# khuongnd6/ViT_torch

Hardware: AMD Instinct MI355X
Metric: images/sec fwd+bwd ViT-B/16 224^2 bs=256/GPU (higher is better)
Workload: dtype bf16; 1 GPU; dino_vitb16 224x224 fwd+CE+bwd+SGD(momentum) step, batch 256/GPU, 10 classes, random-init weights; global_batch=256, residual_stream=bf16, parallelism=dp1, hip_graph=True

## Files before the change

vit_torch_amd/csrc/common.h:

```cpp
#pragma once
#include <hip/hip_runtime.h>
#include <stdint.h>
#include <string>
#include "../../include/vitmi.h"

typedef __bf16 bf16;
typedef bf16 bf16x2 __attribute__((ext_vector_type(2)));
typedef bf16 bf16x4 __attribute__((ext_vector_type(4)));
typedef bf16 bf16x8 __attribute__((ext_vector_type(8)));
typedef float f32x2 __attribute__((ext_vector_type(2)));
typedef float f32x4 __attribute__((ext_vector_type(4)));
typedef float f32x16 __attribute__((ext_vector_type(16)));

#define LDS_PTR(T, p) ((__attribute__((address_space(3))) T*)(p))

void vitmi_set_error(const std::string& s);
int vitmi_fail(int code, const char* fmt, ...);
int vitmi_check_launch(const char* what);
int vitmi_cu_count();
int vitmi_persist_on(int launch_flags);
int vitmi_raise_dynamic_lds(const void* kern, int bytes, const char* who);
int vitmi_reduce_rows(const float* part, int S, int64_t N, int64_t ld, float* out, hipStream_t stream);
int vitmi_reduce_rows_segs(const float* part, int S, int64_t ld, float* const out[4], const int width[4],
                           hipStream_t stream);
int vitmi_reduce_rows3(const float* part, int S, int64_t N, int64_t ld, float* out0, float* out1, float* out2,
                       hipStream_t stream);

#define VITMI_REQUIRE(cond, code, ...)                  \
  do {                                                  \
    if (!(cond)) return vitmi_fail((code), __VA_ARGS__); \
  } while (0)

static inline bool is_aligned(const void* p, size_t a) {
  return (reinterpret_cast<uintptr_t>(p) % a) == 0;
}
static inline size_t dtype_size(int dt) { return dt == VITMI_BF16 ? 2 : 4; }

__device__ __forceinline__ float to_f32(float v) { return v; }
__device__ __forceinline__ float to_f32(bf16 v) { return (float)v; }
template <typename T> __device__ __forceinline__ T from_f32(float v);
template <> __device__ __forceinline__ float from_f32<float>(float v) { return v; }
template <> __device__ __forceinline__ bf16 from_f32<bf16>(float v) { return (bf16)v; }

__device__ __forceinline__ float wave_sum(float v) {
#pragma unroll
  for (int o = 32; o > 0; o >>= 1) v += __shfl_xor(v, o);
  return v;
}
__device__ __forceinline__ float wave_max(float v) {
#pragma unroll
  for (int o = 32; o > 0; o >>= 1) v = fmaxf(v, __shfl_xor(v, o));
  return v;
}

template <int CTRL, int ROW_MASK>
__device__ __forceinline__ float dpp_take(float old, float v) {
  return __builtin_bit_cast(float, __builtin_amdgcn_update_dpp(__builtin_bit_cast(int, old), __builtin_bit_cast(int, v),
                                                               CTRL, ROW_MASK, 0xf, false));
}
__device__ __forceinline__ float wave_sum_dpp(float v) {
  v += dpp_take<0xB1, 0xf>(0.f, v);
  v += dpp_take<0x4E, 0xf>(0.f, v);
  v += dpp_take<0x141, 0xf>(0.f, v);
  v += dpp_take<0x140, 0xf>(0.f, v);
  v += dpp_take<0x142, 0xa>(0.f, v);
  v += dpp_take<0x143, 0xc>(0.f, v);
  return __builtin_bit_cast(float, __builtin_amdgcn_readlane(__builtin_bit_cast(int, v), 63));
}
__device__ __forceinline__ float wave_max_dpp(float v) {
  v = fmaxf(v, dpp_take<0xB1, 0xf>(-INFINITY, v));
  v = fmaxf(v, dpp_take<0x4E, 0xf>(-INFINITY, v));
  v = fmaxf(v, dpp_take<0x141, 0xf>(-INFINITY, v));
  v = fmaxf(v, dpp_take<0x140, 0xf>(-INFINITY, v));
  v = fmaxf(v, dpp_take<0x142, 0xa>(-INFINITY, v));
  v = fmaxf(v, dpp_take<0x143, 0xc>(-INFINITY, v));
  return __builtin_bit_cast(float, __builtin_amdgcn_readlane(__builtin_bit_cast(int, v), 63));
}

__device__ __forceinline__ float gelu_erf(float x) {
  return 0.5f * x * (1.0f + erff(x * 0.70710678118654752440f));
}
__device__ __forceinline__ float dgelu_erf(float x) {
  const float cdf = 0.5f * (1.0f + erff(x * 0.70710678118654752440f));
  const float pdf = 0.39894228040143267794f * __expf(-0.5f * x * x);
  return cdf + x * pdf;
}

template <typename T> __device__ __forceinline__ f32x4 load4(const T* p);
template <> __device__ __forceinline__ f32x4 load4<float>(const float* p) {
  return *reinterpret_cast<const f32x4*>(p);
}
template <> __device__ __forceinline__ f32x4 load4<bf16>(const bf16* p) {
  bf16x4 v = *reinterpret_cast<const bf16x4*>(p);
  f32x4 r = {(float)v[0], (float)v[1], (float)v[2], (float)v[3]};
  return r;
}
template <typename T> __device__ __forceinline__ void store4(T* p, f32x4 v);
template <> __device__ __forceinline__ void store4<float>(float* p, f32x4 v) {
  *reinterpret_cast<f32x4*>(p) = v;
}
template <> __device__ __forceinline__ void store4<bf16>(bf16* p, f32x4 v) {
  bf16x4 r = {(bf16)v[0], (bf16)v[1], (bf16)v[2], (bf16)v[3]};
  *reinterpret_cast<bf16x4*>(p) = r;
}

__device__ __forceinline__ int mfma32_row(int reg, int lane_hi) {
  return (reg & 3) + 8 * (reg >> 2) + 4 * lane_hi;
}
```

vit_torch_amd/csrc/elementwise.hip:

```cpp
#include "common.h"

namespace {

constexpr int EW_BLOCK = 256;
inline unsigned ew_grid(int64_t work_items) {
  int64_t b = (work_items + EW_BLOCK - 1) / EW_BLOCK;
  const int64_t cap = 256 * 8;
  if (b > cap) b = cap;
  if (b < 1) b = 1;
  return (unsigned)b;
}

template <typename TS, typename TD>
__global__ void cast_kernel(const TS* __restrict__ src, TD* __restrict__ dst, int64_t n) {
  const int64_t stride = (int64_t)gridDim.x * blockDim.x;
  const int64_t n4 = n / 4;
  for (int64_t i = (int64_t)blockIdx.x * blockDim.x + threadIdx.x; i < n4; i += stride)
    store4<TD>(dst + i * 4, load4<TS>(src + i * 4));
  for (int64_t i = n4 * 4 + (int64_t)blockIdx.x * blockDim.x + threadIdx.x; i < n; i += stride)
    dst[i] = from_f32<TD>(to_f32(src[i]));
}

__global__ void axpy_kernel(const float* __restrict__ x, float* __restrict__ y, float a, int64_t n) {
  const int64_t stride = (int64_t)gridDim.x * blockDim.x;
// ... 168 lines not shown
  int n;
};
__global__ __launch_bounds__(1024) void fold_many_kernel(FoldTable t) {
  __shared__ float red[FOLD_GROUPS][FOLD_COLS];
  const int b = blockIdx.x;
  int i = 0;
  while (i < t.n - 1 && b >= t.blk_end[i]) ++i;
  const int lb = b - (i ? t.blk_end[i - 1] : 0);
  const int N = t.N[i], cb = (N + FOLD_COLS - 1) / FOLD_COLS;
  const int seg = lb / cb;
  const int64_t c = (int64_t)(lb % cb) * FOLD_COLS + threadIdx.x % FOLD_COLS;
  const float tot = fold_rows(t.part[i], t.S[i], t.ld[i], (int64_t)seg * N + c, c < N, red);
  if (threadIdx.x < FOLD_COLS && c < N) t.out[i][seg][c] = tot;
}

inline int colsum_splits(int64_t M) {
  int64_t s = (M + 3) / 4;
  return (int)(s < 512 ? s : 512);
}

constexpr float XENT_LSE_SWITCH = 16.f;
__global__ __launch_bounds__(256) void xent_kernel(const float* __restrict__ logits,
                                                   const int64_t* __restrict__ labels,
                                                   float* __restrict__ loss_rows,
                                                   float* __restrict__ dlogits,
                                                   int32_t* __restrict__ correct_rows,
                                                   int64_t B, int K) {
  const int lane = threadIdx.x & 63, w = threadIdx.x >> 6;
  const int64_t b = (int64_t)blockIdx.x * 4 + w;
  if (b >= B) return;
  const float* lr = logits + b * K;
  float mx = -INFINITY;
  int amax = 0;
  for (int k = lane; k < K; k += 64) {
    const float v = lr[k];
    if (v > mx) { mx = v; amax = k; }
  }
#pragma unroll
  for (int o = 32; o > 0; o >>= 1) {
    const float om = __shfl_xor(mx, o);
    const int oa = __shfl_xor(amax, o);
    if (om > mx || (om == mx && oa < amax)) { mx = om; amax = oa; }
  }
  float se = 0.f;
  for (int k = lane; k < K; k += 64) se += __expf(lr[k] - mx);
  se = wave_sum(se);
  const float lg = __logf(se);
  const float lse = mx + lg;
  const bool rel = !(fabsf(lse) < XENT_LSE_SWITCH);
  const int64_t lab = labels[b];
  const float invB = 1.f / (float)B;
  if (dlogits) {
    for (int k = lane; k < K; k += 64) {
      const float p = rel ? __expf((lr[k] - mx) - lg) : __expf(lr[k] - lse);
      dlogits[b * K + k] = (p - (k == lab ? 1.f : 0.f)) * invB;
    }
  }
  if (lane == 0) {
    const bool ok = lab >= 0 && lab < (int64_t)K;
    const float xl = lr[ok ? lab : 0];
    loss_rows[b] = ok ? (rel ? lg - (xl - mx) : lse - xl) : __builtin_nanf("");
    correct_rows[b] = (ok && amax == (int)lab) ? 1 : 0;
  }
}

__global__ __launch_bounds__(256) void xent_reduce_kernel(const float* __restrict__ loss_rows,
                                                          const int32_t* __restrict__ correct_rows,
                                                          float* __restrict__ loss,
                                                          int32_t* __restrict__ correct, int64_t B) {
  __shared__ float sl[256];
  __shared__ int sc[256];
  float l = 0.f;
  int c = 0;
  for (int64_t i = threadIdx.x; i < B; i += 256) { l += loss_rows[i]; c += correct_rows[i]; }
  sl[threadIdx.x] = l; sc[threadIdx.x] = c;
  __syncthreads();
  for (int o = 128; o > 0; o >>= 1) {
    if ((int)threadIdx.x < o) { sl[threadIdx.x] += sl[threadIdx.x + o]; sc[threadIdx.x] += sc[threadIdx.x + o]; }
    __syncthreads();
  }
  if (threadIdx.x == 0) { loss[0] = sl[0] / (float)B; if (correct) correct[0] = sc[0]; }
}

__global__ void sgd_momentum_kernel(float* __restrict__ p, const float* __restrict__ g,
                                    float* __restrict__ buf, bf16* __restrict__ shadow, int64_t n,
                                    float lr, float momentum, float gscale) {
  const int64_t stride = (int64_t)gridDim.x * blockDim.x;
  const int64_t n4 = n / 4;
  for (int64_t i = (int64_t)blockIdx.x * blockDim.x + threadIdx.x; i < n4; i += stride) {
    const f32x4 gv = __builtin_nontemporal_load(reinterpret_cast<const f32x4*>(g + i * 4));
    f32x4 bv = __builtin_nontemporal_load(reinterpret_cast<const f32x4*>(buf + i * 4));
    f32x4 pv = __builtin_nontemporal_load(reinterpret_cast<const f32x4*>(p + i * 4));
#pragma unroll
    for (int e = 0; e < 4; ++e) {
      bv[e] = momentum * bv[e] + gscale * gv[e];
      pv[e] = pv[e] - lr * bv[e];
    }
    __builtin_nontemporal_store(bv, reinterpret_cast<f32x4*>(buf + i * 4));
    __builtin_nontemporal_store(pv, reinterpret_cast<f32x4*>(p + i * 4));
    if (shadow) store4<bf16>(shadow + i * 4, pv);
  }
  for (int64_t i = n4 * 4 + (int64_t)blockIdx.x * blockDim.x + threadIdx.x; i < n; i += stride) {
    const float b = momentum * buf[i] + gscale * g[i];
    buf[i] = b;
    const float pn = p[i] - lr * b;
    p[i] = pn;
    if (shadow) shadow[i] = (bf16)pn;
  }
}

__global__ void adam_tick_kernel(float* state) { state[0] += 1.f; }

__global__ void adam_kernel(float* __restrict__ p, const float* __restrict__ g, float* __restrict__ m,
                            float* __restrict__ v, bf16* __restrict__ shadow, const float* __restrict__ state,
                            int64_t n, float lr, float b1, float b2, float eps, float wd, int decoupled,
                            float gscale) {
  const double t = state[0];
  const double bc1 = 1.0 - pow((double)b1, t), bc2 = 1.0 - pow((double)b2, t);
  const float step = (float)((double)lr / bc1), bc2s = (float)sqrt(bc2);
  const float lrwd = decoupled ? (float)((double)lr * (double)wd) : 0.f;
  const int64_t stride = (int64_t)gridDim.x * blockDim.x;
  for (int64_t i = (int64_t)blockIdx.x * blockDim.x + threadIdx.x; i < n; i += stride) {
    float pi = p[i], gi = g[i] * gscale;
    if (!decoupled) gi = fmaf(wd, pi, gi);
    const float mi = b1 * m[i] + (1.f - b1) * gi;
    const float vi = b2 * v[i] + (1.f - b2) * gi * gi;
    m[i] = mi;
    v[i] = vi;
    pi -= fmaf(lrwd, pi, step * mi / (sqrtf(vi) / bc2s + eps));
    p[i] = pi;
    if (shadow) shadow[i] = (bf16)pi;
  }
}

}

int vitmi_reduce_rows3(const float* part, int S, int64_t N, int64_t ld, float* out0, float* out1, float* out2,
                       hipStream_t stream) {
  const unsigned segs = out2 ? 3 : 2;
  hipLaunchKernelGGL(reduce_rows3_kernel, dim3((unsigned)((N + FOLD_COLS - 1) / FOLD_COLS), segs), dim3(1024), 0, stream, part, S,
                     N, ld, out0, out1, out2);
  return vitmi_check_launch("reduce_rows3_kernel");
}

int vitmi_reduce_rows_segs(const float* part, int S, int64_t ld, float* const out[4], const int width[4],
                           hipStream_t stream) {
  RowSegs sg;
  int e = 0;
  for (int i = 0; i < 4; ++i) { sg.out[i] = out[i]; e += width[i]; sg.end[i] = e; }
  hipLaunchKernelGGL(reduce_rows_segs_kernel, dim3((unsigned)((e + FOLD_COLS - 1) / FOLD_COLS)), dim3(1024), 0, stream, part, S, ld, sg);
  return vitmi_check_launch("reduce_rows_segs_kernel");
}

extern "C" int vitmi_fold_many(const vitmi_fold_desc* descs, int n, void* stream_) {
  VITMI_REQUIRE(descs && n > 0, VITMI_E_BADARG, "fold_many: null descriptors or n <= 0");
  hipStream_t stream = reinterpret_cast<hipStream_t>(stream_);
  for (int i0 = 0; i0 < n; i0 += FOLD_MAX) {
    FoldTable t;
    t.n = n - i0 < FOLD_MAX ? n - i0 : FOLD_MAX;
    int blocks = 0;
    for (int i = 0; i < FOLD_MAX; ++i) {
      const vitmi_fold_desc& d = descs[i0 + (i < t.n ? i : 0)];
      if (i < t.n) {
        VITMI_REQUIRE(d.struct_size == (int64_t)sizeof(vitmi_fold_desc), VITMI_E_BADARG, "fold_many: descriptor size %lld, this library expects %zu", (long long)d.struct_size, sizeof(vitmi_fold_desc));
        VITMI_REQUIRE(d.part && d.S > 0 && d.nseg >= 1 && d.nseg <= 3 && d.N > 0 && d.N < (1ll << 30) && d.ld >= d.nseg * d.N && d.ld < (1ll << 31),
                      VITMI_E_SHAPE, "fold_many: descriptor %d: S %d, nseg %d, N %lld, ld %lld", i0 + i, d.S, d.nseg, (long long)d.N, (long long)d.ld);
        for (int k = 0; k < d.nseg; ++k) VITMI_REQUIRE(d.out[k], VITMI_E_BADARG, "fold_many: descriptor %d: null output %d", i0 + i, k);
        blocks += d.nseg * (int)((d.N + FOLD_COLS - 1) / FOLD_COLS);
      }
      t.part[i] = d.part; t.S[i] = d.S; t.N[i] = (int)d.N; t.ld[i] = (int)d.ld; t.blk_end[i] = blocks;
      for (int k = 0; k < 3; ++k) t.out[i][k] = d.out[k < d.nseg ? k : 0];
    }
// ... 58 lines not shown
  if (out_ld <= 0) out_ld = C * p * p;
  VITMI_REQUIRE(out_ld >= C * p * p && out_ld % 4 == 0, VITMI_E_BADARG, "patchify: out_ld must be >= C*p*p and a multiple of 4");
  VITMI_REQUIRE(is_aligned(out, 4 * dtype_size(out_dtype)), VITMI_E_ALIGN, "patchify: out alignment");
  hipStream_t stream = reinterpret_cast<hipStream_t>(stream_);
  const int64_t ntok = cls_rows + (H / p) * (W / p);
  const int64_t total = B * ntok * (out_ld / 4);
  const unsigned grid = ew_grid(total);
  if (out_dtype == VITMI_BF16)
    hipLaunchKernelGGL((patchify_kernel<bf16>), dim3(grid), dim3(EW_BLOCK), 0, stream, x, sb, sc, sh, sw, (bf16*)out, out_ld, B, (int)C, (int)H, (int)W, (int)p, cls_rows);
  else if (out_dtype == VITMI_F32)
    hipLaunchKernelGGL((patchify_kernel<float>), dim3(grid), dim3(EW_BLOCK), 0, stream, x, sb, sc, sh, sw, (float*)out, out_ld, B, (int)C, (int)H, (int)W, (int)p, cls_rows);
  else return vitmi_fail(VITMI_E_DTYPE, "patchify: bad out dtype");
  return vitmi_check_launch("patchify_kernel");
}

extern "C" size_t vitmi_colsum_workspace(int64_t M, int64_t N) {
  return (size_t)colsum_splits(M) * (size_t)N * sizeof(float);
}

extern "C" int vitmi_colsum(const void* x, int dtype, int64_t M, int64_t N, int64_t ld, float* out,
                            void* workspace, size_t workspace_bytes, void* stream_) {
  VITMI_REQUIRE(x && out && M > 0 && N > 0 && ld >= N, VITMI_E_BADARG, "colsum: bad argument");
  VITMI_REQUIRE(workspace && workspace_bytes >= vitmi_colsum_workspace(M, N), VITMI_E_WORKSPACE, "colsum: workspace too small");
  hipStream_t stream = reinterpret_cast<hipStream_t>(stream_);
  if (dtype == VITMI_F32 && M <= 2048) return vitmi_reduce_rows(reinterpret_cast<const float*>(x), (int)M, N, ld, out, stream);
  const int S = colsum_splits(M);
  float* part = reinterpret_cast<float*>(workspace);
  const bool vec = (N % 4 == 0) && (ld % 4 == 0) && is_aligned(x, 4 * dtype_size(dtype));
  if (vec && N <= 512 && (dtype == VITMI_BF16 || dtype == VITMI_F32)) {
    const int gpr = (int)(N / 4);
    if (dtype == VITMI_BF16) hipLaunchKernelGGL((colsum_partial_rows_kernel<bf16>), dim3((unsigned)S), dim3(256), 0, stream, (const bf16*)x, M, gpr, ld, part);
    else hipLaunchKernelGGL((colsum_partial_rows_kernel<float>), dim3((unsigned)S), dim3(256), 0, stream, (const float*)x, M, gpr, ld, part);
    int rc = vitmi_check_launch("colsum_partial_rows_kernel");
    if (rc) return rc;
    return vitmi_reduce_rows(part, S, N, N, out, stream);
  }
  const int cols_per_block = vec ? 256 : 64;
  dim3 grid((unsigned)((N + cols_per_block - 1) / cols_per_block), (unsigned)S);
  if (dtype == VITMI_BF16) {
    if (vec) hipLaunchKernelGGL((colsum_partial_kernel<bf16, 4>), grid, dim3(256), 0, stream, (const bf16*)x, M, N, ld, part);
    else hipLaunchKernelGGL((colsum_partial_kernel<bf16, 1>), grid, dim3(256), 0, stream, (const bf16*)x, M, N, ld, part);
  } else if (dtype == VITMI_F32) {
    if (vec) hipLaunchKernelGGL((colsum_partial_kernel<float, 4>), grid, dim3(256), 0, stream, (const float*)x, M, N, ld, part);
    else hipLaunchKernelGGL((colsum_partial_kernel<float, 1>), grid, dim3(256), 0, stream, (const float*)x, M, N, ld, part);
  } else return vitmi_fail(VITMI_E_DTYPE, "colsum: bad dtype");
  int rc = vitmi_check_launch("colsum_partial_kernel");
  if (rc) return rc;
  return vitmi_reduce_rows(part, S, N, N, out, stream);
}

extern "C" int vitmi_softmax_xent(const float* logits, const int64_t* labels, float* loss,
                                  float* dlogits, int32_t* correct, int64_t B, int64_t K,
                                  void* stream_) {
  VITMI_REQUIRE(logits && labels && loss && B > 0 && K > 0, VITMI_E_BADARG, "softmax_xent: bad argument");
  VITMI_REQUIRE(dlogits, VITMI_E_BADARG, "softmax_xent: dlogits buffer required (its tail is used as scratch)");
  VITMI_REQUIRE(correct, VITMI_E_BADARG, "softmax_xent: correct buffer required");
  hipStream_t stream = reinterpret_cast<hipStream_t>(stream_);
  hipLaunchKernelGGL(xent_kernel, dim3((unsigned)((B + 3) / 4)), dim3(256), 0, stream, logits, labels, loss + 1, dlogits, correct + 1, B, (int)K);
  int rc = vitmi_check_launch("xent_kernel");
  if (rc) return rc;
  hipLaunchKernelGGL(xent_reduce_kernel, dim3(1), dim3(256), 0, stream, loss + 1, correct + 1, loss, correct, B);
  return vitmi_check_launch("xent_reduce_kernel");
}

extern "C" int vitmi_adam(float* p, const float* g, float* m, float* v, void* shadow, float* state, int64_t n,
                          float lr, float beta1, float beta2, float eps, float weight_decay, int decoupled,
                          float grad_scale, void* stream_) {
  VITMI_REQUIRE(p && g && m && v && state && n > 0, VITMI_E_BADARG, "adam: bad argument");
  VITMI_REQUIRE(beta1 >= 0.f && beta1 < 1.f && beta2 >= 0.f && beta2 < 1.f && eps >= 0.f, VITMI_E_BADARG, "adam: bad hyper-parameter");
  hipStream_t stream = reinterpret_cast<hipStream_t>(stream_);
  hipLaunchKernelGGL(adam_tick_kernel, dim3(1), dim3(1), 0, stream, state);
  int rc = vitmi_check_launch("adam_tick_kernel");
  if (rc) return rc;
  hipLaunchKernelGGL(adam_kernel, dim3(ew_grid(n)), dim3(EW_BLOCK), 0, stream, p, g, m, v, (bf16*)shadow, state, n, lr,
                     beta1, beta2, eps, weight_decay, decoupled, grad_scale);
  return vitmi_check_launch("adam_kernel");
}

extern "C" int vitmi_sgd_momentum(float* p, const float* g, float* buf, void* shadow, int64_t n,
                                  float lr, float momentum, float grad_scale, void* stream_) {
  VITMI_REQUIRE(p && g && buf && n > 0, VITMI_E_BADARG, "sgd_momentum: bad argument");
  VITMI_REQUIRE(is_aligned(p, 16) && is_aligned(g, 16) && is_aligned(buf, 16) && (!shadow || is_aligned(shadow, 8)), VITMI_E_ALIGN, "sgd_momentum: buffers must be 16-B aligned");
  hipStream_t stream = reinterpret_cast<hipStream_t>(stream_);
  hipLaunchKernelGGL(sgd_momentum_kernel, dim3(ew_grid(n / 4 + 1)), dim3(EW_BLOCK), 0, stream, p, g, buf, (bf16*)shadow, n, lr, momentum, grad_scale);
  return vitmi_check_launch("sgd_momentum_kernel");
}
```

vit_torch_amd/csrc/layernorm.hip:

```cpp
#include <atomic>
#include <initializer_list>
#include "common.h"

namespace {

constexpr int LN_MAXV = 8;

template <int NV, typename TX, typename TY>
__global__ __launch_bounds__(256) void ln_fwd_kernel(const TX* __restrict__ x, int64_t xs,
                                                     const float* __restrict__ gamma,
                                                     const float* __restrict__ beta,
                                                     TY* __restrict__ y, int64_t ys,
                                                     float* __restrict__ mean_out,
                                                     float* __restrict__ rstd_out,
                                                     int64_t M, int D, float eps) {
  const int lane = threadIdx.x & 63, w = threadIdx.x >> 6;
  for (int64_t row = (int64_t)blockIdx.x * 4 + w; row < M; row += (int64_t)gridDim.x * 4) {
  const TX* xr = x + row * xs;
  f32x4 v[NV];
  float s = 0.f;
#pragma unroll
  for (int i = 0; i < NV; ++i) v[i] = load4<TX>(xr + min((i * 64 + lane) * 4, D - 4));
#pragma unroll
  for (int i = 0; i < NV; ++i) {
// ... 81 lines not shown
          dv[i][j] *= gam[i][j];
          s1 += dv[i][j];
          s2 += dv[i][j] * xh[i][j];
        }
      }
    }
    const float c1 = wave_sum(s1) * invD, c2 = wave_sum(s2) * invD;
    float rsc = 1.f;
    if (gb_rowscale) rsc = gb_rowscale[(uint32_t)row / (uint32_t)rpg];
    f32x4 gin[NV];
    if (g_in) {
#pragma unroll
      for (int i = 0; i < NV; ++i) gin[i] = load4<TG>(g_in + row * gstride + min((i * 64 + lane) * 4, D - 4));
    }
#pragma unroll
    for (int i = 0; i < NV; ++i) {
      const int c = (i * 64 + lane) * 4;
      if (c < D) {
        f32x4 o;
#pragma unroll
        for (int j = 0; j < 4; ++j) o[j] = rs * (dv[i][j] - c1 - xh[i][j] * c2);
        if (g_in) {
#pragma unroll
          for (int j = 0; j < 4; ++j) o[j] += gin[i][j];
        }
        store4<TG>(g_out + row * gstride + c, o);
        if (gb_scale) {
          const f32x4 sc = *reinterpret_cast<const f32x4*>(gb_scale + c);
#pragma unroll
          for (int j = 0; j < 4; ++j) o[j] *= sc[j];
        }
        if (gb_rowscale) {
#pragma unroll
          for (int j = 0; j < 4; ++j) o[j] *= rsc;
        }
        if (gb_out) store4<TGB>(gb_out + row * gbs + c, o);
#pragma unroll
        for (int j = 0; j < 4; ++j) gs[i][j] += o[j];
      }
    }
  }
  float* prow = part + (int64_t)blockIdx.x * 3 * D;
#pragma unroll 1
  for (int pass = 0; pass < (want_gsum ? 3 : 2); ++pass) {
#pragma unroll
    for (int i = 0; i < NV; ++i) {
      const int c = (i * 64 + lane) * 4;
      if (c < D) *reinterpret_cast<f32x4*>(red + w * D + c) = pass == 0 ? dg[i] : (pass == 1 ? db[i] : gs[i]);
    }
    __syncthreads();
    for (int c = threadIdx.x; c < D; c += 256)
      prow[pass * D + c] = (red[c] + red[D + c]) + (red[2 * D + c] + red[3 * D + c]);
    __syncthreads();
  }
}

template <typename T> __device__ __forceinline__ void load8(const T* p, float (&o)[8]);
template <> __device__ __forceinline__ void load8<float>(const float* p, float (&o)[8]) {
  const f32x4 a = *reinterpret_cast<const f32x4*>(p), b = *reinterpret_cast<const f32x4*>(p + 4);
  o[0] = a[0]; o[1] = a[1]; o[2] = a[2]; o[3] = a[3]; o[4] = b[0]; o[5] = b[1]; o[6] = b[2]; o[7] = b[3];
}
template <> __device__ __forceinline__ void load8<bf16>(const bf16* p, float (&o)[8]) {
  const bf16x8 v = *reinterpret_cast<const bf16x8*>(p);
#pragma unroll
  for (int i = 0; i < 8; ++i) o[i] = (float)v[i];
}
template <typename T> __device__ __forceinline__ void store8(T* p, const float (&v)[8]);
template <> __device__ __forceinline__ void store8<float>(float* p, const float (&v)[8]) {
  *reinterpret_cast<f32x4*>(p) = f32x4{v[0], v[1], v[2], v[3]};
  *reinterpret_cast<f32x4*>(p + 4) = f32x4{v[4], v[5], v[6], v[7]};
}
template <> __device__ __forceinline__ void store8<bf16>(bf16* p, const float (&v)[8]) {
  bf16x8 o;
#pragma unroll
  for (int i = 0; i < 8; ++i) o[i] = (bf16)v[i];
  *reinterpret_cast<bf16x8*>(p) = o;
}
template <int LPR> __device__ __forceinline__ float group_sum(float v) {
#pragma unroll
  for (int o = LPR / 2; o > 0; o >>= 1) v += __shfl_xor(v, o);
  return v;
}

template <int LPR, int NV, typename TX, typename TY>
__global__ __launch_bounds__(256) void ln_fwd8_kernel(const TX* __restrict__ x, int64_t xs, const float* __restrict__ gamma,
                                                      const float* __restrict__ beta, TY* __restrict__ y, int64_t ys,
                                                      float* __restrict__ mean_out, float* __restrict__ rstd_out,
                                                      int64_t M, int D, float eps) {
  constexpr int RPW = 64 / LPR;
  const int lane = threadIdx.x & 63, w = threadIdx.x >> 6;
  const int sub = lane / LPR, l = lane % LPR;
  const int64_t groups = (M + RPW - 1) / RPW;
  const float invD = 1.f / (float)D;
  for (int64_t grp = (int64_t)blockIdx.x * 4 + w; grp < groups; grp += (int64_t)gridDim.x * 4) {
    const int64_t row = grp * RPW + sub;
    const bool live = row < M;
    const TX* xr = x + (live ? row : M - 1) * xs;
    float v[NV][8];
#pragma unroll
    for (int i = 0; i < NV; ++i) load8<TX>(xr + min((i * LPR + l) * 8, D - 8), v[i]);
    float s = 0.f;
#pragma unroll
    for (int i = 0; i < NV; ++i)
      if ((i * LPR + l) * 8 < D) {
#pragma unroll
        for (int j = 0; j < 8; ++j) s += v[i][j];
      }
    const float mean = group_sum<LPR>(s) * invD;
    float q = 0.f;
#pragma unroll
    for (int i = 0; i < NV; ++i)
      if ((i * LPR + l) * 8 < D) {
#pragma unroll
        for (int j = 0; j < 8; ++j) { const float d = v[i][j] - mean; q += d * d; }
      }
    const float rstd = rsqrtf(group_sum<LPR>(q) * invD + eps);
    if (l == 0 && live) {
      if (mean_out) mean_out[row] = mean;
      if (rstd_out) rstd_out[row] = rstd;
    }
    TY* yr = y + row * ys;
#pragma unroll
    for (int i = 0; i < NV; ++i) {
      const int c = (i * LPR + l) * 8;
      float g[8], b[8];
      load8<float>(gamma + min(c, D - 8), g);
      load8<float>(beta + min(c, D - 8), b);
      if (c < D && live) {
        float o[8];
#pragma unroll
        for (int j = 0; j < 8; ++j) o[j] = (v[i][j] - mean) * rstd * g[j] + b[j];
        store8<TY>(yr + c, o);
      }
    }
  }
}

template <int LPR, int NV, typename TDY, typename TX, typename TG, typename TGB>
__global__ __launch_bounds__(256) void ln_bwd8_kernel(const TDY* __restrict__ dy, int64_t dys, const TX* __restrict__ x, int64_t xs,
                                                      const float* __restrict__ mean, const float* __restrict__ rstd,
                                                      const float* __restrict__ gamma, const TG* g_in, TG* g_out, int64_t gstride,
                                                      TGB* __restrict__ gb_out, int64_t gbs, float* __restrict__ part, int want_gsum,
                                                      const float* __restrict__ gb_scale, const float* __restrict__ gb_rowscale,
                                                      int64_t rpg, int64_t M, int D) {
  extern __shared__ __attribute__((aligned(16))) float red[];
  constexpr int RPW = 64 / LPR;
  const int lane = threadIdx.x & 63, w = threadIdx.x >> 6;
  const int sub = lane / LPR, l = lane % LPR;
  float gam[NV][8], dg[NV][8], db[NV][8], gs[NV][8];
#pragma unroll
  for (int i = 0; i < NV; ++i) {
    load8<float>(gamma + min((i * LPR + l) * 8, D - 8), gam[i]);
#pragma unroll
    for (int j = 0; j < 8; ++j) { dg[i][j] = 0.f; db[i][j] = 0.f; gs[i][j] = 0.f; }
  }
  const float invD = 1.f / (float)D;
  const int64_t groups = (M + RPW - 1) / RPW;
  for (int64_t grp = (int64_t)blockIdx.x * 4 + w; grp < groups; grp += (int64_t)gridDim.x * 4) {
    const int64_t row = grp * RPW + sub;
    const bool live = row < M;
    const int64_t r = live ? row : M - 1;
    const float mu = mean[r], rs = rstd[r];
    float xh[NV][8], dv[NV][8], gin[NV][8];
#pragma unroll
    for (int i = 0; i < NV; ++i) {
      const int cc = min((i * LPR + l) * 8, D - 8);
      load8<TX>(x + r * xs + cc, xh[i]);
      load8<TDY>(dy + r * dys + cc, dv[i]);
    }
    if (g_in) {
#pragma unroll
      for (int i = 0; i < NV; ++i) load8<TG>(g_in + r * gstride + min((i * LPR + l) * 8, D - 8), gin[i]);
    }
    float s1 = 0.f, s2 = 0.f;
#pragma unroll
    for (int i = 0; i < NV; ++i)
      if ((i * LPR + l) * 8 < D && live) {
#pragma unroll
        for (int j = 0; j < 8; ++j) {
          xh[i][j] = (xh[i][j] - mu) * rs;
          dg[i][j] += dv[i][j] * xh[i][j];
          db[i][j] += dv[i][j];
          dv[i][j] *= gam[i][j];
          s1 += dv[i][j];
          s2 += dv[i][j] * xh[i][j];
        }
      }
    const float c1 = group_sum<LPR>(s1) * invD, c2 = group_sum<LPR>(s2) * invD;
    float rsc = 1.f;
    if (gb_rowscale) rsc = gb_rowscale[(uint32_t)r / (uint32_t)rpg];
#pragma unroll
    for (int i = 0; i < NV; ++i) {
      const int c = (i * LPR + l) * 8;
      if (c < D && live) {
        float o[8];
#pragma unroll
        for (int j = 0; j < 8; ++j) o[j] = rs * (dv[i][j] - c1 - xh[i][j] * c2);
        if (g_in) {
#pragma unroll
          for (int j = 0; j < 8; ++j) o[j] += gin[i][j];
        }
        store8<TG>(g_out + row * gstride + c, o);
        if (gb_scale) {
          float sc[8];
          load8<float>(gb_scale + c, sc);
#pragma unroll
          for (int j = 0; j < 8; ++j) o[j] *= sc[j];
        }
        if (gb_rowscale) {
#pragma unroll
          for (int j = 0; j < 8; ++j) o[j] *= rsc;
        }
        if (gb_out) store8<TGB>(gb_out + row * gbs + c, o);
#pragma unroll
        for (int j = 0; j < 8; ++j) gs[i][j] += o[j];
      }
    }
// ... 1 lines not shown
  float* prow = part + (int64_t)blockIdx.x * 3 * D;
  const int slot = w * RPW + sub;
#pragma unroll 1
  for (int pass = 0; pass < (want_gsum ? 3 : 2); ++pass) {
#pragma unroll
    for (int i = 0; i < NV; ++i) {
      const int c = (i * LPR + l) * 8;
      float t[8];
#pragma unroll
      for (int j = 0; j < 8; ++j) t[j] = pass == 0 ? dg[i][j] : (pass == 1 ? db[i][j] : gs[i][j]);
      if (c < D) store8<float>(red + slot * D + c, t);
    }
    __syncthreads();
    for (int c = threadIdx.x; c < D; c += 256) {
      float a = 0.f;
#pragma unroll
      for (int t = 0; t < 4 * RPW; ++t) a += red[t * D + c];
      prow[pass * D + c] = a;
    }
    __syncthreads();
  }
}

struct Ln8Cfg { int lpr, nv; };
inline Ln8Cfg ln8_cfg(int64_t D) {
  if (D <= 128) return {16, 1};
  if (D <= 256) return {16, 2};
  if (D <= 384) return {16, 3};
  if (D <= 512) return {32, 2};
  if (D <= 768) return {32, 3};
  if (D <= 1024) return {64, 2};
  if (D <= 1536) return {64, 3};
  return {64, 4};
}
static std::atomic<int> g_ln8{1};

inline int ln_nv(int64_t D) { return D <= 512 ? 2 : D <= 768 ? 3 : D <= 1024 ? 4 : LN_MAXV; }
inline int ln_bwd_blocks(int64_t M, int64_t D) {
  const int nv = ln_nv(D);
  const int64_t cap = nv == 2 ? 1024 : nv <= 4 ? 768 : 512;
  int64_t b = (M + 3) / 4;
  return (int)(b < cap ? b : cap);
}

inline bool ln8_ok(int64_t D, std::initializer_list<int64_t> strides, std::initializer_list<const void*> ptrs) {
  if (!g_ln8 || D % 8 != 0 || D < 8) return false;
  for (int64_t s : strides) if (s % 8 != 0) return false;
  for (const void* p : ptrs) if (p && !is_aligned(p, 16)) return false;
  return true;
}
inline int ln_bwd8_blocks(int64_t M, int64_t D) {
  const Ln8Cfg c = ln8_cfg(D);
  const int64_t groups = (M + 64 / c.lpr - 1) / (64 / c.lpr);
  const int64_t cap = c.nv == 1 ? 1024 : c.nv == 2 ? 768 : c.nv == 3 ? 512 : 256;
  const int64_t b = (groups + 3) / 4;
  return (int)(b < cap ? b : cap);
}

}

extern "C" void vitmi_debug_ln8(int on) { g_ln8 = on != 0; }

static int check_ln_common(const void* x, int x_dtype, int64_t x_stride, int64_t M, int64_t D, const char* who) {
  VITMI_REQUIRE(x && M > 0 && D > 0, VITMI_E_BADARG, "%s: null input or empty shape", who);
  VITMI_REQUIRE(D % 4 == 0 && D <= LN_MAXV * 256, VITMI_E_SHAPE, "%s: D=%lld must be a multiple of 4 and <= %d", who, (long long)D, LN_MAXV * 256);
  VITMI_REQUIRE(x_stride % 4 == 0 && is_aligned(x, 4 * dtype_size(x_dtype)), VITMI_E_ALIGN, "%s: rows must be 4-element aligned", who);
  return 0;
}

extern "C" int vitmi_layernorm_fwd(const void* x, int x_dtype, int64_t x_stride, const float* gamma,
                                   const float* beta, void* y, int y_dtype, int64_t y_stride,
                                   float* mean, float* rstd, int64_t M, int64_t D, float eps,
                                   void* stream_) {
  int rc = check_ln_common(x, x_dtype, x_stride, M, D, "layernorm_fwd");
  if (rc) return rc;
  VITMI_REQUIRE(y && gamma && beta, VITMI_E_BADARG, "layernorm_fwd: null y/gamma/beta");
  VITMI_REQUIRE(y_stride % 4 == 0 && is_aligned(y, 4 * dtype_size(y_dtype)) && is_aligned(gamma, 16) && is_aligned(beta, 16),
                VITMI_E_ALIGN, "layernorm_fwd: y/gamma/beta alignment");
  hipStream_t stream = reinterpret_cast<hipStream_t>(stream_);
  if (ln8_ok(D, {x_stride, y_stride}, {x, y, gamma, beta})) {
    const Ln8Cfg c = ln8_cfg(D);
    const int rpw = 64 / c.lpr;
    int64_t nb = ((M + rpw - 1) / rpw + 3) / 4;
    if (nb > 2048) nb = 2048;
#define LN_FWD8_T(L, N, TX, TY)                                                                                  \
    hipLaunchKernelGGL((ln_fwd8_kernel<L, N, TX, TY>), dim3((unsigned)nb), dim3(256), 0, stream, (const TX*)x, x_stride, \
                       gamma, beta, (TY*)y, y_stride, mean, rstd, M, (int)D, eps)
#define LN_FWD8(TX, TY)                                                                  \
    do {                                                                                  \
      switch (c.lpr * 8 + c.nv) {                                                         \
        case 16 * 8 + 1: LN_FWD8_T(16, 1, TX, TY); break;                                 \
        case 16 * 8 + 2: LN_FWD8_T(16, 2, TX, TY); break;                                 \
        case 16 * 8 + 3: LN_FWD8_T(16, 3, TX, TY); break;                                 \
        case 32 * 8 + 2: LN_FWD8_T(32, 2, TX, TY); break;                                 \
        case 32 * 8 + 3: LN_FWD8_T(32, 3, TX, TY); break;                                 \
        case 64 * 8 + 2: LN_FWD8_T(64, 2, TX, TY); break;                                 \
        case 64 * 8 + 3: LN_FWD8_T(64, 3, TX, TY); break;                                 \
        default: LN_FWD8_T(64, 4, TX, TY); break;                                         \
      }                                                                                   \
    } while (0)
    if (x_dtype == VITMI_F32 && y_dtype == VITMI_F32) LN_FWD8(float, float);
    else if (x_dtype == VITMI_F32 && y_dtype == VITMI_BF16) LN_FWD8(float, bf16);
    else if (x_dtype == VITMI_BF16 && y_dtype == VITMI_BF16) LN_FWD8(bf16, bf16);
    else if (x_dtype == VITMI_BF16 && y_dtype == VITMI_F32) LN_FWD8(bf16, float);
    else return vitmi_fail(VITMI_E_DTYPE, "layernorm_fwd: dtype combination");
#undef LN_FWD8
#undef LN_FWD8_T
    return vitmi_check_launch("ln_fwd8_kernel");
  }
  int64_t nblk = (M + 3) / 4;
  if (nblk > 2048) nblk = 2048;
  dim3 grid((unsigned)nblk), block(256);
#define LN_FWD_NV(NVV, TX, TY)                                                                     \
  hipLaunchKernelGGL((ln_fwd_kernel<NVV, TX, TY>), grid, block, 0, stream, (const TX*)x, x_stride, \
                     gamma, beta, (TY*)y, y_stride, mean, rstd, M, (int)D, eps)
#define LN_FWD(TX, TY)                                                                        \
  do {                                                                                        \
    switch (ln_nv(D)) {                                                                       \
      case 2: LN_FWD_NV(2, TX, TY); break;                                                    \
      case 3: LN_FWD_NV(3, TX, TY); break;                                                    \
      case 4: LN_FWD_NV(4, TX, TY); break;                                                    \
      default: LN_FWD_NV(LN_MAXV, TX, TY); break;                                             \
    }                                                                                         \
  } while (0)
  if (x_dtype == VITMI_F32 && y_dtype == VITMI_F32) LN_FWD(float, float);
  else if (x_dtype == VITMI_F32 && y_dtype == VITMI_BF16) LN_FWD(float, bf16);
  else if (x_dtype == VITMI_BF16 && y_dtype == VITMI_BF16) LN_FWD(bf16, bf16);
  else if (x_dtype == VITMI_BF16 && y_dtype == VITMI_F32) LN_FWD(bf16, float);
  else return vitmi_fail(VITMI_E_DTYPE, "layernorm_fwd: dtype combination");
#undef LN_FWD
#undef LN_FWD_NV
  return vitmi_check_launch("ln_fwd_kernel");
}

extern "C" size_t vitmi_layernorm_bwd_workspace(int64_t M, int64_t D) {
  int nb = ln_bwd_blocks(M, D);
  if (D % 8 == 0 && D >= 8) nb = nb > ln_bwd8_blocks(M, D) ? nb : ln_bwd8_blocks(M, D);
  return (size_t)nb * 3 * (size_t)D * sizeof(float);
}

extern "C" int vitmi_layernorm_bwd(const void* dy, int dy_dtype, int64_t dy_stride, const void* x,
                                   int x_dtype, int64_t x_stride, const float* mean,
                                   const float* rstd, const float* gamma, const void* g_in,
                                   void* g_out, int g_dtype, int64_t g_stride, void* gb_out,
                                   int gb_dtype, int64_t gb_stride, float* dgamma, float* dbeta,
                                   float* gsum, const float* gb_scale, const float* gb_rowscale,
                                   int64_t rows_per_group, int64_t M, int64_t D,
                                   void* workspace, size_t workspace_bytes, void* stream_) {
  vitmi_fold_desc fold;
  int rc = vitmi_layernorm_bwd_deferred(dy, dy_dtype, dy_stride, x, x_dtype, x_stride, mean, rstd, gamma, g_in, g_out, g_dtype,
                                        g_stride, gb_out, gb_dtype, gb_stride, dgamma, dbeta, gsum, gb_scale, gb_rowscale,
                                        rows_per_group, M, D, workspace, workspace_bytes, &fold, stream_);
  if (rc) return rc;
  return vitmi_fold_many(&fold, 1, stream_);
}

static void ln_fold_desc(vitmi_fold_desc* f, const float* part, int S, int64_t D, float* dgamma, float* dbeta, float* gsum) {
  f->struct_size = (int64_t)sizeof(vitmi_fold_desc);
  f->part = part; f->S = S; f->nseg = gsum ? 3 : 2; f->N = D; f->ld = 3 * D;
  f->out[0] = dgamma; f->out[1] = dbeta; f->out[2] = gsum;
}

extern "C" int vitmi_layernorm_bwd_deferred(const void* dy, int dy_dtype, int64_t dy_stride, const void* x,
                                            int x_dtype, int64_t x_stride, const float* mean,
                                            const float* rstd, const float* gamma, const void* g_in,
                                            void* g_out, int g_dtype, int64_t g_stride, void* gb_out,
                                            int gb_dtype, int64_t gb_stride, float* dgamma, float* dbeta,
                                            float* gsum, const float* gb_scale, const float* gb_rowscale,
// ... 90 lines not shown
```

Baseline: 8136 images/sec.

## Prefetch next LayerNorm row, hoist gamma/beta, size grids by resident occupancy

The LayerNorm forward kernel now loads gamma/beta once per wave and software-pipelines the input rows, issuing the next row's loads before reducing the current one. Its grid is capped at the number of resident blocks from an occupancy query instead of a fixed 2048. The SGD momentum kernel is unrolled 4x with batched loads and launched with an occupancy-sized grid. The aim is to hide memory latency in these bandwidth-bound kernels, at the cost of more registers and a one-time occupancy query on the host.

After: 8164 images/sec, median of 6. About the same (+0.3%).

```diff
diff --git a/vit_torch_amd/csrc/common.h b/vit_torch_amd/csrc/common.h
--- a/vit_torch_amd/csrc/common.h
+++ b/vit_torch_amd/csrc/common.h
@@ -1,6 +1,7 @@
 #pragma once
 #include <hip/hip_runtime.h>
 #include <stdint.h>
+#include <atomic>
 #include <string>
 #include "../../include/vitmi.h"
 
@@ -35,6 +36,15 @@
   return (reinterpret_cast<uintptr_t>(p) % a) == 0;
 }
 static inline size_t dtype_size(int dt) { return dt == VITMI_BF16 ? 2 : 4; }
+
+template <typename K> static inline int64_t vitmi_resident_blocks(K kernel, int threads, std::atomic<int>& per_cu) {
+  int n = per_cu.load(std::memory_order_relaxed);
+  if (n <= 0) {
+    if (hipOccupancyMaxActiveBlocksPerMultiprocessor(&n, kernel, threads, 0) != hipSuccess || n <= 0) return 0;
+    per_cu.store(n, std::memory_order_relaxed);
+  }
+  return (int64_t)n * vitmi_cu_count();
+}
 
 __device__ __forceinline__ float to_f32(float v) { return v; }
 __device__ __forceinline__ float to_f32(bf16 v) { return (float)v; }
diff --git a/vit_torch_amd/csrc/elementwise.hip b/vit_torch_amd/csrc/elementwise.hip
--- a/vit_torch_amd/csrc/elementwise.hip
+++ b/vit_torch_amd/csrc/elementwise.hip
@@ -274,12 +274,35 @@
   if (threadIdx.x == 0) { loss[0] = sl[0] / (float)B; if (correct) correct[0] = sc[0]; }
 }
 
+constexpr int SGD_UNROLL = 4;
 __global__ void sgd_momentum_kernel(float* __restrict__ p, const float* __restrict__ g,
                                     float* __restrict__ buf, bf16* __restrict__ shadow, int64_t n,
                                     float lr, float momentum, float gscale) {
   const int64_t stride = (int64_t)gridDim.x * blockDim.x;
   const int64_t n4 = n / 4;
-  for (int64_t i = (int64_t)blockIdx.x * blockDim.x + threadIdx.x; i < n4; i += stride) {
+  int64_t i = (int64_t)blockIdx.x * blockDim.x + threadIdx.x;
+  constexpr int U = SGD_UNROLL;
+  for (; i + (U - 1) * stride < n4; i += U * stride) {
+    f32x4 gv[U], bv[U], pv[U];
+#pragma unroll
+    for (int u = 0; u < U; ++u) gv[u] = __builtin_nontemporal_load(reinterpret_cast<const f32x4*>(g + (i + u * stride) * 4));
+#pragma unroll
+    for (int u = 0; u < U; ++u) bv[u] = __builtin_nontemporal_load(reinterpret_cast<const f32x4*>(buf + (i + u * stride) * 4));
+#pragma unroll
+    for (int u = 0; u < U; ++u) pv[u] = __builtin_nontemporal_load(reinterpret_cast<const f32x4*>(p + (i + u * stride) * 4));
+#pragma unroll
+    for (int u = 0; u < U; ++u) {
+#pragma unroll
+      for (int e = 0; e < 4; ++e) {
+        bv[u][e] = momentum * bv[u][e] + gscale * gv[u][e];
+        pv[u][e] = pv[u][e] - lr * bv[u][e];
+      }
+      __builtin_nontemporal_store(bv[u], reinterpret_cast<f32x4*>(buf + (i + u * stride) * 4));
+      __builtin_nontemporal_store(pv[u], reinterpret_cast<f32x4*>(p + (i + u * stride) * 4));
+      if (shadow) store4<bf16>(shadow + (i + u * stride) * 4, pv[u]);
+    }
+  }
+  for (; i < n4; i += stride) {
     const f32x4 gv = __builtin_nontemporal_load(reinterpret_cast<const f32x4*>(g + i * 4));
     f32x4 bv = __builtin_nontemporal_load(reinterpret_cast<const f32x4*>(buf + i * 4));
     f32x4 pv = __builtin_nontemporal_load(reinterpret_cast<const f32x4*>(p + i * 4));
@@ -504,6 +527,11 @@
   VITMI_REQUIRE(p && g && buf && n > 0, VITMI_E_BADARG, "sgd_momentum: bad argument");
   VITMI_REQUIRE(is_aligned(p, 16) && is_aligned(g, 16) && is_aligned(buf, 16) && (!shadow || is_aligned(shadow, 8)), VITMI_E_ALIGN, "sgd_momentum: buffers must be 16-B aligned");
   hipStream_t stream = reinterpret_cast<hipStream_t>(stream_);
-  hipLaunchKernelGGL(sgd_momentum_kernel, dim3(ew_grid(n / 4 + 1)), dim3(EW_BLOCK), 0, stream, p, g, buf, (bf16*)shadow, n, lr, momentum, grad_scale);
+  static std::atomic<int> per_cu{0};
+  const int64_t cap = vitmi_resident_blocks(sgd_momentum_kernel, EW_BLOCK, per_cu);
+  VITMI_REQUIRE(cap > 0, VITMI_E_BADARG, "sgd_momentum: the occupancy query of sgd_momentum_kernel failed");
+  int64_t nb = n / 4 / (EW_BLOCK * SGD_UNROLL);
+  nb = nb < 1 ? 1 : nb > cap ? cap : nb;
+  hipLaunchKernelGGL(sgd_momentum_kernel, dim3((unsigned)nb), dim3(EW_BLOCK), 0, stream, p, g, buf, (bf16*)shadow, n, lr, momentum, grad_scale);
   return vitmi_check_launch("sgd_momentum_kernel");
 }
diff --git a/vit_torch_amd/csrc/layernorm.hip b/vit_torch_amd/csrc/layernorm.hip
--- a/vit_torch_amd/csrc/layernorm.hip
+++ b/vit_torch_amd/csrc/layernorm.hip
@@ -187,6 +187,23 @@
   return v;
 }
 
+template <typename T> struct Raw8;
+template <> struct Raw8<float> { f32x4 a, b; };
+template <> struct Raw8<bf16> { bf16x8 v; };
+__device__ __forceinline__ Raw8<float> load8_raw(const float* p) {
+  return {*reinterpret_cast<const f32x4*>(p), *reinterpret_cast<const f32x4*>(p + 4)};
+}
+__device__ __forceinline__ Raw8<bf16> load8_raw(const bf16* p) { return {*reinterpret_cast<const bf16x8*>(p)}; }
+__device__ __forceinline__ void unpack8(const Raw8<float>& r, float (&o)[8]) {
+  o[0] = r.a[0]; o[1] = r.a[1]; o[2] = r.a[2]; o[3] = r.a[3]; o[4] = r.b[0]; o[5] = r.b[1]; o[6] = r.b[2]; o[7] = r.b[3];
+}
+__device__ __forceinline__ void unpack8(const Raw8<bf16>& r, float (&o)[8]) {
+#pragma unroll
+  for (int i = 0; i < 8; ++i) o[i] = (float)r.v[i];
+}
+
+constexpr int LN_WAIT_VM0 = 0x0f70;
+
 template <int LPR, int NV, typename TX, typename TY>
 __global__ __launch_bounds__(256) void ln_fwd8_kernel(const TX* __restrict__ x, int64_t xs, const float* __restrict__ gamma,
                                                       const float* __restrict__ beta, TY* __restrict__ y, int64_t ys,
@@ -196,14 +213,37 @@
   const int lane = threadIdx.x & 63, w = threadIdx.x >> 6;
   const int sub = lane / LPR, l = lane % LPR;
   const int64_t groups = (M + RPW - 1) / RPW;
+  const int64_t stride = (int64_t)gridDim.x * 4;
+  int64_t grp = (int64_t)blockIdx.x * 4 + w;
+  if (grp >= groups) return;
   const float invD = 1.f / (float)D;
-  for (int64_t grp = (int64_t)blockIdx.x * 4 + w; grp < groups; grp += (int64_t)gridDim.x * 4) {
+  float g[NV][8], b[NV][8];
+  Raw8<TX> nx[NV];
+#pragma unroll
+  for (int i = 0; i < NV; ++i) {
+    const int cc = min((i * LPR + l) * 8, D - 8);
+    load8<float>(gamma + cc, g[i]);
+    load8<float>(beta + cc, b[i]);
+  }
+  {
+    const TX* xr = x + min(grp * RPW + sub, M - 1) * xs;
+#pragma unroll
+    for (int i = 0; i < NV; ++i) nx[i] = load8_raw(xr + min((i * LPR + l) * 8, D - 8));
+  }
+  __builtin_amdgcn_s_waitcnt(LN_WAIT_VM0);
+  for (;;) {
     const int64_t row = grp * RPW + sub;
     const bool live = row < M;
-    const TX* xr = x + (live ? row : M - 1) * xs;
     float v[NV][8];
 #pragma unroll
-    for (int i = 0; i < NV; ++i) load8<TX>(xr + min((i * LPR + l) * 8, D - 8), v[i]);
+    for (int i = 0; i < NV; ++i) unpack8(nx[i], v[i]);
+    const int64_t nxt = grp + stride;
+    const bool more = nxt < groups;
+    if (more) {
+      const TX* xr = x + min(nxt * RPW + sub, M - 1) * xs;
+#pragma unroll
+      for (int i = 0; i < NV; ++i) nx[i] = load8_raw(xr + min((i * LPR + l) * 8, D - 8));
+    }
     float s = 0.f;
 #pragma unroll
     for (int i = 0; i < NV; ++i)
@@ -228,16 +268,15 @@
 #pragma unroll
     for (int i = 0; i < NV; ++i) {
       const int c = (i * LPR + l) * 8;
-      float g[8], b[8];
-      load8<float>(gamma + min(c, D - 8), g);
-      load8<float>(beta + min(c, D - 8), b);
       if (c < D && live) {
         float o[8];
 #pragma unroll
-        for (int j = 0; j < 8; ++j) o[j] = (v[i][j] - mean) * rstd * g[j] + b[j];
+        for (int j = 0; j < 8; ++j) o[j] = (v[i][j] - mean) * rstd * g[i][j] + b[i][j];
         store8<TY>(yr + c, o);
       }
     }
+    if (!more) break;
+    grp = nxt;
   }
 }
 
@@ -405,8 +444,13 @@
     const Ln8Cfg c = ln8_cfg(D);
     const int rpw = 64 / c.lpr;
     int64_t nb = ((M + rpw - 1) / rpw + 3) / 4;
-    if (nb > 2048) nb = 2048;
 #define LN_FWD8_T(L, N, TX, TY)                                                                                  \
+    {                                                                                                             \
+      static std::atomic<int> per_cu{0};                                                                          \
+      const int64_t cap = vitmi_resident_blocks(ln_fwd8_kernel<L, N, TX, TY>, 256, per_cu);                       \
+      VITMI_REQUIRE(cap > 0, VITMI_E_BADARG, "layernorm_fwd: the occupancy query of ln_fwd8_kernel failed");      \
+      if (nb > cap) nb = cap;                                                                                     \
+    }                                                                                                             \
     hipLaunchKernelGGL((ln_fwd8_kernel<L, N, TX, TY>), dim3((unsigned)nb), dim3(256), 0, stream, (const TX*)x, x_stride, \
                        gamma, beta, (TY*)y, y_stride, mean, rstd, M, (int)D, eps)
 #define LN_FWD8(TX, TY)                                                                  \
```
